# linhthi/BLISS-GNN

Measured on AMD Instinct MI355X. Metric: steps/sec (train step: sample_blocks + gather + SAGE fwd/bwd + Adam + exp3), reddit-like, higher is better.
Workload: dtype bf16

## Files before the change

### bliss_gnn_amd/_lib.py

```python
import ctypes as C
import os

_HERE = os.path.dirname(os.path.abspath(__file__))
LIB_PATH = os.path.join(_HERE, "libbliss_gnn.so")

EINVAL = -1
MODE_BANDIT, MODE_LADIES, MODE_UNIFORM_NODES, MODE_PARTIALS = 0, 1, 4, 8
WIDE_MAX_K = 16384
NR_MAX_FANOUT = 1024
WN_RAW, WN_EXP3 = 0, 1

ERR_BITS = {
    1: "frontier larger than 2^31-1 edges",
    2: "candidate capacity exceeded / seed id out of range",
    4: "kept-node capacity exceeded",
    8: "block-edge capacity exceeded",
    16: "non-finite or negative weight reached an exact reduction",
    32: "exact sum left its fixed-point range",
    64: "seed capacity exceeded",
    128: "random stream ran short / generator made no progress",
    256: "a cross-stream flag never came (bliss_flag_wait timed out)",
}


# ... 259 lines not shown
    "bliss_spmm_bwd": [_P, _P, _P, _P, _P, _P, _P, _I64, _I32, _P, _I32, _I32, C.c_int, _P, _I64, C.c_int, _P, _P],
    "bliss_spmm_max_fwd": [_P, _P, _P, _P, _P, _I64, _I32, _P, _I32, _I32, _P, _I64, _P, _I64, _P, _P],
    "bliss_spmm_max_bwd": [_P, _P, _P, _P, _P, _P, _I64, _P, _I64, _I32, _P, _I32, _I32, _P, _I64, _P, _P],
    "bliss_spmm_max_bwd_relu": [_P, _P, _P, _P, _P, _P, _I64, _P, _I64, _P, _I64, _I32, _P, _I32, _I32, _P, _I64, _P, _P],
    "bliss_spmm_self_fwd": [_P, _P, _P, _P, _P, _I64, _P, _I64, _I32, _P, _P, _I32, _I32, _P, _I64, _P, _P],
    "bliss_spmm_self_bwd": [_P, _P, _P, _P, _P, _P, _P, _I64, _I32, _I32, _P, _P, _I32, _I32, _P, _I64, _P, _P],
    "bliss_sddmm_dot": [_P, _P, _P, _P, _I32, _P, _I64, _P, _I64, _P, _I64, _I32, _I32, _P, _I32, _P],
    "bliss_lstm_tile_rows": [],
    "bliss_lstm_agg_fwd": [_P, _P, _P, _P, _I64, _P, _I64, _P, _P, _I32, _P, _P, _I32, _I32, _P, _I64, _P, _P, _P, _P],
    "bliss_lstm_agg_bwd": [_P, _P, _I64, _P, _I64, _P, _P, _I32, _P, _P, _I32, _I32, _P, _P],
    "bliss_lstm_edge_reduce": [_P, _P, _P, _P, _I32, _P, _I32, _I32, _P, _I64, _P],
    "bliss_block_transpose": [_P, _P, _I32, _I32, _I32, _P, _P, _P, _I64, _P],
    "bliss_spmm_chunk_edges": [_I32],
    "bliss_sage_epilogue_fwd": [_P, _I64, _P, _I64, _I32, _I32, _F, C.c_uint32, _P, _P, _I64, _P, _P],
    "bliss_sage_epilogue_bwd": [_P, _I64, _P, _I64, _I32, _I32, _F, _P, _I64, _P],
    "bliss_gat_chunk_edges": [],
    "bliss_graph_prepare": [_P, _P, _I64, _I32, C.c_int, _P, _P, _P, _P, _P, _P, _I64, _P],
    "bliss_exp3_update": [C.POINTER(Graph), _P, _P, _P, _P, _P, _P, _P, _P, _P, _P, _P, _P, _I32, _P, _I32, _F, _P, _P, C.c_int, _P, _P],
    "bliss_exp3_step": [C.POINTER(Graph), _P, C.POINTER(Exp3Block), _I32, _F, _P, _P],
    "bliss_exp3_normalize_global_rows": [C.POINTER(Exp3Block), _I32, _I64, _P, _I64, _P],
    "bliss_exp3_update_blocks": [C.POINTER(Graph), _P, C.POINTER(Exp3Block), _I32, _F, _P, _P],
    "bliss_exp3_apply": [_P, _P, _P, _P, _P, _I32, _P, _P],
    "bliss_exp3_normalize": [_P, _I64, _P, _P, _P, _P],
    "bliss_row_sum": [_P, _I64, _P, _P],
    "bliss_gat_logits": [_P, _P, _P, _I32, _P, _I64, _P, _I32, _I32, _F, _P, _P],
    "bliss_sage_dgrad": [C.POINTER(DGrad), _P],
    "bliss_sage_wgrad": [C.POINTER(WGrad), _I32, _P, _I64, _P],
    "bliss_gat_dgrad": [C.POINTER(DGrad), _P],
    "bliss_dgrad_wide": [C.POINTER(DGrad), _P],
    "bliss_gat_glue_fwd": [C.POINTER(GatGlue), _P],
# ... 105 lines not shown
```

### bliss_gnn_amd/csrc/prof.h

```cpp
#pragma once
#include <hip/hip_runtime.h>

enum BlissKernelId {
  BK_SEG_SCAN = 0, BK_PASS1, BK_PASS2, BK_CHUNK_SCAN, BK_PASS3, BK_CAND_FINALIZE, BK_POISSON_SCALE, BK_SELECT1, BK_SELECT2,
  BK_BLOCK1, BK_INDPTR_SCAN, BK_BLOCK2, BK_CLEANUP, BK_MT19937, BK_SPMM_FWD, BK_SPMM_BWD, BK_EMBED_NORM, BK_EXP3_UPDATE,
  BK_EXP3_APPLY, BK_NORMALIZE, BK_ROW_SUM, BK_NORM_EDATA, BK_TRANSPOSE, BK_SPMM_FIXUP, BK_SPMM_MAX_FWD, BK_SPMM_MAX_FIXUP,
  BK_SPMM_MAX_BWD, BK_SPMM_MAX_BWD_FIXUP, BK_COL_SUMS, BK_BIN_SCATTER, BK_BIN_REDUCE, BK_BITMAP_SCAN, BK_CAND_NUMBER,
  BK_SPMM_SELF_FWD, BK_SPMM_SELF_FIXUP, BK_SPMM_SELF_BWD, BK_SPMM_SELF_BWD_FIXUP,
  BK_LSTM_AGG_FWD, BK_LSTM_AGG_BWD, BK_LSTM_EDGE_REDUCE,
  BK_SDDMM_DOT,
  BK_SPMM_MAX_BWD_RELU, BK_SPMM_MAX_BWD_RELU_FIXUP, BK_COUNT
};

extern int g_bliss_prof_sel;
void bliss_prof_begin(int id, hipStream_t st);
void bliss_prof_end(int id, hipStream_t st);

#define PROF_LAUNCH(id, st, ...)                                              \
  do {                                                                        \
    const bool p_ = (g_bliss_prof_sel == -1 || g_bliss_prof_sel == (id));    \
    if (p_) bliss_prof_begin((id), (st));                                     \
    __VA_ARGS__;                                                              \
    if (p_) bliss_prof_end((id), (st));                                       \
  } while (0)
// ... 1 lines not shown
```

### bliss_gnn_amd/csrc/prof.hip

```cpp
#include "prof.h"
#include "bliss_gnn.h"
#include <mutex>
#include <vector>

int g_bliss_prof_sel = -2;

namespace {
struct Pair { hipEvent_t a, b; int id; };
std::mutex g_mu;
std::vector<Pair> g_open, g_free;
double g_ms[BK_COUNT];
long long g_n[BK_COUNT];
const char* kNames[BK_COUNT] = {
  "k_seg_scan", "k_frontier_pass1", "k_frontier_pass2", "k_chunk_scan", "k_frontier_pass3", "k_cand_finalize", "k_poisson_scale",
  "k_select_pass1", "k_select_pass2", "k_block_pass1", "k_indptr_scan", "k_block_pass2", "k_cleanup", "k_mt19937_uniform",
  "k_spmm_fwd", "k_spmm_bwd", "k_embed_norm", "k_exp3_update", "k_exp3_apply", "k_normalize_row", "k_row_sum",
  "k_normalized_edata", "k_block_transpose", "k_spmm_fixup", "k_spmm_max", "k_spmm_max_fixup", "k_spmm_max_bwd",
  "k_spmm_max_bwd_fixup", "k_col_sums", "k_bin_scatter", "k_bin_reduce", "k_bitmap_scan", "k_cand_number",
  "k_spmm_self", "k_spmm_self_fixup", "k_spmm_self_bwd", "k_spmm_self_bwd_fixup",
  "k_lstm_agg_fwd", "k_lstm_agg_bwd", "k_lstm_edge_reduce", "k_sddmm_dot",
  "k_spmm_max_bwd_relu", "k_spmm_max_bwd_relu_fixup"};
thread_local Pair t_cur;

void drain_locked() {
  for (auto& p : g_open) {
    (void)hipEventSynchronize(p.b);
    float ms = 0.f;
    if (hipEventElapsedTime(&ms, p.a, p.b) == hipSuccess) { g_ms[p.id] += ms; g_n[p.id] += 1; }
    g_free.push_back(p);
  }
  g_open.clear();
}
}

void bliss_prof_begin(int id, hipStream_t st) {
// ... 47 lines not shown
```

### bliss_gnn_amd/csrc/spmm.hip

```cpp
#include "common.cuh"
#include "spmm_walk.cuh"
#include "bliss_gnn.h"
#include "prof.h"

namespace {

using namespace spmm_walk;

#define SP_TPB 256

template <bool BWD>
struct SagePolicy {
  const int* blk_indptr;
  int mean;
  __device__ __forceinline__ float coef(float c, int s, int d) const {
    if (BWD && mean) c = c / (float)max(blk_indptr[d + 1] - blk_indptr[d], 1);
    return c;
  }
  __device__ __forceinline__ float scale(int r, int rb, int re) const {
    return (!BWD && mean) ? 1.0f / (float)max(re - rb, 1) : 1.0f;
  }
};

template <bool VEC4, bool OUT_F32, bool BWD>
// ... 61 lines not shown
  __builtin_amdgcn_fence(__ATOMIC_RELEASE, "wavefront");
  __builtin_amdgcn_wave_barrier();
  float s = 0.f;
  if (norm_vec4) {
    for (int c = lane * 4; c < dim; c += 256) {
      const float a = bf2f(sh[c]), b = bf2f(sh[c + 1]), cc = bf2f(sh[c + 2]), d = bf2f(sh[c + 3]);
      s += a * a; s += b * b; s += cc * cc; s += d * d;
    }
  } else {
    for (int c = lane; c < dim; c += 64) { const float a = bf2f(sh[c]); s += a * a; }
  }
  for (int d = 32; d >= 1; d >>= 1) s += __shfl_xor(s, d);
  if (lane == 0) norm_out[row] = f2bf(sqrtf(s));
}

template <bool VEC4, bool NORM4>
__global__ void __launch_bounds__(SP_TPB) k_sage_epilogue(const bf16_t* __restrict__ a, int64_t a_stride, const bf16_t* __restrict__ b,
                                                         int64_t b_stride, int n_rows, int dim, uint32_t drop_thresh, float scale,
                                                         uint32_t seed, unsigned long long* ctr, bf16_t* __restrict__ out,
                                                         int64_t out_stride, bf16_t* __restrict__ norm_out) {
  const int lane = lane_id();
  const int row = blockIdx.x * (SP_TPB / 64) + (threadIdx.x >> 6);
  const uint32_t c = drop_thresh ? (uint32_t)__hip_atomic_load(ctr, __ATOMIC_RELAXED, __HIP_MEMORY_SCOPE_AGENT) : 0u;
  if (row < n_rows) {
    const bf16_t *pa = a + row * a_stride, *pb = b + row * b_stride;
    bf16_t* po = out + row * out_stride;
    float s = 0.f;
    static_assert(NORM4 || !VEC4, "8-byte accesses imply the vec4 order");
    constexpr int W = NORM4 ? 4 : 1;
    for (int col = lane * W; col < dim; col += 64 * W) {
      float v[W];
      if (VEC4) {
        const f4 x = load4(pa + col), y = load4(pb + col);
        v[0] = x.x + y.x; v[1 % W] = x.y + y.y; v[2 % W] = x.z + y.z; v[3 % W] = x.w + y.w;
      } else {
#pragma unroll
        for (int i = 0; i < W; ++i) v[i] = bf2f(pa[col + i]) + bf2f(pb[col + i]);
      }
#pragma unroll
      for (int i = 0; i < W; ++i) {
        float t = rbf(v[i]);
        t = t > 0.f ? t : 0.f;
        if (drop_thresh) {
          const bool keep = drop_hash(seed, c, (uint32_t)(row * dim + col + i)) >= drop_thresh;
          t = keep ? rbf(t * scale) : 0.f;
        }
        v[i] = t;
        s += t * t;
      }
      if (VEC4) {
        uint2 o;
        o.x = (uint32_t)f2bf(v[0]) | ((uint32_t)f2bf(v[1 % W]) << 16);
        o.y = (uint32_t)f2bf(v[2 % W]) | ((uint32_t)f2bf(v[3 % W]) << 16);
        *reinterpret_cast<uint2*>(po + col) = o;
      } else {
#pragma unroll
        for (int i = 0; i < W; ++i) po[col + i] = f2bf(v[i]);
      }
    }
    for (int d = 32; d >= 1; d >>= 1) s += __shfl_xor(s, d);
    if (lane == 0 && norm_out) norm_out[row] = f2bf(sqrtf(s));
  }
  if (drop_thresh) {
    __syncthreads();
    if (threadIdx.x == 0) {
      const unsigned G = gridDim.x < 64u ? gridDim.x : 64u, g = blockIdx.x % G;
      const unsigned long long members = (gridDim.x - g + G - 1) / G;
      if (atomicAdd(ctr + 2 + g, 1ull) == members - 1) {
        __hip_atomic_store(ctr + 2 + g, 0ull, __ATOMIC_RELAXED, __HIP_MEMORY_SCOPE_AGENT);
        if (atomicAdd(ctr + 1, 1ull) == (unsigned long long)G - 1) {
          __hip_atomic_store(ctr + 1, 0ull, __ATOMIC_RELAXED, __HIP_MEMORY_SCOPE_AGENT);
          atomicAdd(ctr, 1ull);
        }
      }
    }
  }
}

template <bool VEC4>
__global__ void __launch_bounds__(SP_TPB) k_sage_epilogue_bwd(const bf16_t* __restrict__ dout, int64_t d_stride, const bf16_t* __restrict__ out,
                                                             int64_t out_stride, int n_rows, int dim, float scale,
                                                             bf16_t* __restrict__ din, int64_t din_stride) {
  const int lane = lane_id();
  const int row = blockIdx.x * (SP_TPB / 64) + (threadIdx.x >> 6);
  if (row >= n_rows) return;
  constexpr int W = VEC4 ? 4 : 1;
  for (int col = lane * W; col < dim; col += 64 * W) {
    if (VEC4) {
      const f4 g = load4(dout + row * d_stride + col), o = load4(out + row * out_stride + col);
      f4 r;
      r.x = o.x > 0.f ? g.x * scale : 0.f; r.y = o.y > 0.f ? g.y * scale : 0.f;
      r.z = o.z > 0.f ? g.z * scale : 0.f; r.w = o.w > 0.f ? g.w * scale : 0.f;
      store4<false>(din, row * din_stride + col, r);
    } else {
      const float g = bf2f(dout[row * d_stride + col]);
      din[row * din_stride + col] = f2bf(bf2f(out[row * out_stride + col]) > 0.f ? g * scale : 0.f);
    }
  }
}

template <bool BWD>
int launch_spmm(const int* row_ptr, const int* t_edge, const int* src, const int* dst, const int* blk_indptr, const void* w,
                const void* h, int64_t h_stride, int n_rows, const int* nnz_dev, int nnz, int dim, int mean, void* out,
                int64_t out_stride, int out_fp32, float* part, hipStream_t st) {
  if (n_rows <= 0 || dim <= 0) return 0;
  const int EC = spmm_chunk_edges(nnz);
  if (nnz > EC && !part) return BLISS_EINVAL;
  const bool vec4 = (dim % 4 == 0) && (h_stride % 4 == 0) && (out_stride % 4 == 0) &&
                    (((uintptr_t)h) % 8 == 0) && (((uintptr_t)out) % (out_fp32 ? 16 : 8) == 0);
  const int nchunks = nnz > 0 ? (nnz + EC - 1) / EC : 1;
  dim3 grid((nchunks + SP_TPB / 64 - 1) / (SP_TPB / 64)), block(SP_TPB), gfix((n_rows + SP_TPB / 64 - 1) / (SP_TPB / 64));
#define GO(V, F) PROF_LAUNCH(BWD ? BK_SPMM_BWD : BK_SPMM_FWD, st, k_spmm<V, F, BWD><<<grid, block, 0, st>>>(row_ptr, t_edge, src, dst, blk_indptr, (const bf16_t*)w, (const bf16_t*)h, h_stride, n_rows, nnz_dev, nnz, dim, mean, out, out_stride, part, EC))
  if (vec4) { if (out_fp32) GO(true, true); else GO(true, false); }
  else      { if (out_fp32) GO(false, true); else GO(false, false); }
#undef GO
  {
    const bool fv = vec4 && (((uintptr_t)part) % 16 == 0);
#define FIX(F, V) PROF_LAUNCH(BK_SPMM_FIXUP, st, k_spmm_fixup<F, BWD, V><<<gfix, block, 0, st>>>(row_ptr, n_rows, dim, mean, part, out, out_stride, EC))
    if (out_fp32) { if (fv) FIX(true, true); else FIX(true, false); }
    else          { if (fv) FIX(false, true); else FIX(false, false); }
#undef FIX
  }
  return (int)hipGetLastError();
}

}

extern "C" {

int bliss_spmm_chunk_edges(int32_t nnz_bound) { return spmm_chunk_edges(nnz_bound); }

// ... 15 lines not shown
}

int bliss_sage_epilogue_fwd(const void* a, int64_t a_stride, const void* b, int64_t b_stride, int32_t n_rows, int32_t dim,
                            float p_drop, uint32_t seed, uint64_t* ctr, void* out, int64_t out_stride, void* norm_out, void* stream) {
  if (!a || !b || !out || n_rows < 0 || dim <= 0 || !(p_drop >= 0.f && p_drop < 1.f) || (p_drop > 0.f && !ctr)) return BLISS_EINVAL;
  if (n_rows == 0) return 0;
  const bool v4 = dim % 4 == 0 && a_stride % 4 == 0 && b_stride % 4 == 0 && out_stride % 4 == 0 && ((uintptr_t)a) % 8 == 0 &&
                  ((uintptr_t)b) % 8 == 0 && ((uintptr_t)out) % 8 == 0;
  const uint32_t thresh = p_drop > 0.f ? (uint32_t)((double)p_drop * 4294967296.0) : 0u;
  const float scale = p_drop > 0.f ? 1.0f / (1.0f - p_drop) : 1.0f;
  hipStream_t st = (hipStream_t)stream;
  const int grid = (n_rows + SP_TPB / 64 - 1) / (SP_TPB / 64);
  const bool n4 = dim % 4 == 0 && out_stride % 4 == 0 && ((uintptr_t)out) % 8 == 0;
#define GO(V, N) k_sage_epilogue<V, N><<<grid, SP_TPB, 0, st>>>((const bf16_t*)a, a_stride, (const bf16_t*)b, b_stride, n_rows, dim, thresh, scale, \
                                                              seed, (unsigned long long*)ctr, (bf16_t*)out, out_stride, (bf16_t*)norm_out)
  if (v4) GO(true, true); else if (n4) GO(false, true); else GO(false, false);
#undef GO
  return (int)hipGetLastError();
}

int bliss_sage_epilogue_bwd(const void* dout, int64_t dout_stride, const void* out, int64_t out_stride, int32_t n_rows, int32_t dim,
                            float p_drop, void* din, int64_t din_stride, void* stream) {
  if (!dout || !out || !din || n_rows < 0 || dim <= 0 || !(p_drop >= 0.f && p_drop < 1.f)) return BLISS_EINVAL;
  if (n_rows == 0) return 0;
  const bool v4 = dim % 4 == 0 && dout_stride % 4 == 0 && out_stride % 4 == 0 && din_stride % 4 == 0 && ((uintptr_t)dout) % 8 == 0 &&
                  ((uintptr_t)out) % 8 == 0 && ((uintptr_t)din) % 8 == 0;
  const float scale = p_drop > 0.f ? 1.0f / (1.0f - p_drop) : 1.0f;
  hipStream_t st = (hipStream_t)stream;
  const int grid = (n_rows + SP_TPB / 64 - 1) / (SP_TPB / 64);
  if (v4) k_sage_epilogue_bwd<true><<<grid, SP_TPB, 0, st>>>((const bf16_t*)dout, dout_stride, (const bf16_t*)out, out_stride, n_rows, dim, scale,
// ... 36 lines not shown
```

### bliss_gnn_amd/csrc/spmm_walk.cuh

```cuda
#pragma once
#include "common.cuh"

namespace spmm_walk {

struct f4 { float x, y, z, w; };

__device__ __forceinline__ int bcast_i(int v, int j) { return __builtin_amdgcn_readlane(v, j); }
__device__ __forceinline__ float bcast_f(float v, int j) { return __int_as_float(__builtin_amdgcn_readlane(__float_as_int(v), j)); }

__device__ __forceinline__ f4 load4(const bf16_t* p) {
  uint2 v = *reinterpret_cast<const uint2*>(p);
  f4 r;
  r.x = __uint_as_float(v.x << 16); r.y = __uint_as_float(v.x & 0xffff0000u);
  r.z = __uint_as_float(v.y << 16); r.w = __uint_as_float(v.y & 0xffff0000u);
  return r;
}

template <bool OUT_F32>
__device__ __forceinline__ void store4(void* out, int64_t off, f4 a) {
  if (OUT_F32) {
    *reinterpret_cast<float4*>((float*)out + off) = make_float4(a.x, a.y, a.z, a.w);
  } else {
    uint2 v;
    v.x = (uint32_t)f2bf(a.x) | ((uint32_t)f2bf(a.y) << 16);
    v.y = (uint32_t)f2bf(a.z) | ((uint32_t)f2bf(a.w) << 16);
    *reinterpret_cast<uint2*>((bf16_t*)out + off) = v;
  }
}

template <bool VEC4, bool OUT_F32>
__device__ __forceinline__ void store_row(void* out, int64_t off, f4 a, float scale) {
  a.x *= scale; a.y *= scale; a.z *= scale; a.w *= scale;
  if (VEC4) store4<OUT_F32>(out, off, a);
  else if (OUT_F32) ((float*)out)[off] = a.x;
  else ((bf16_t*)out)[off] = f2bf(a.x);
}

__host__ __device__ inline int spmm_chunk_edges(int nnz) { return nnz >= 200000 ? 64 : (nnz >= 50000 ? 32 : 16); }

template <bool VEC4, bool OUT_F32, bool BWD, class Policy>
__device__ __forceinline__ void chunk(const Policy pol, int ci, int nnz, int EC, const int* __restrict__ row_ptr,
                                      const int* __restrict__ t_edge, const int* __restrict__ src, const int* __restrict__ dst,
                                      const bf16_t* __restrict__ w, const bf16_t* __restrict__ h, int64_t h_stride, int dim,
                                      void* out, int64_t out_stride, float* __restrict__ part) {
  const int lane = lane_id();
  const int c0 = ci * EC, c1 = min(nnz, c0 + EC), cnt = c1 - c0;
  int my_row = -1, my_n = 0;
  float my_c = 0.f;
  if (lane < cnt) {
    const int e = BWD ? t_edge[c0 + lane] : c0 + lane;
    const int s = src[e], d = dst[e];
    my_row = BWD ? s : d;
    my_n = BWD ? d : s;
    my_c = pol.coef(w ? bf2f(w[e]) : 1.0f, s, d);
  }
  constexpr int W = VEC4 ? 4 : 1;
  const f4 zero = {0.f, 0.f, 0.f, 0.f};
  for (int col0 = 0; col0 < dim; col0 += 64 * W) {
    const int col = col0 + lane * W;
    const bool act = col < dim;
    auto flush = [&](int r, f4 acc) {
      const int rb = row_ptr[r], re = row_ptr[r + 1];
      const bool starts = rb >= c0, ends = re <= c1;
      if (!act) return;
      if (starts && ends) {
        store_row<VEC4, OUT_F32>(out, r * out_stride + col, acc, pol.scale(r, rb, re));
      } else {
        float* q = part + ((int64_t)ci * 2 + (starts ? 1 : 0)) * dim + col;
        q[0] = acc.x;
        if (VEC4) { q[1] = acc.y; q[2] = acc.z; q[3] = acc.w; }
      }
    };
    if (cnt == 0) continue;
    int cur = bcast_i(my_row, 0);
    f4 acc = zero;
    for (int j = 0; j < cnt;) {
      const int r = bcast_i(my_row, j);
      if (r != cur) { flush(cur, acc); acc = zero; cur = r; }
      const int run = __popcll(__ballot(my_row == r && lane >= j));
      const int end = j + run;
      for (; j + 4 <= end; j += 4) {
        int n0 = bcast_i(my_n, j), n1 = bcast_i(my_n, j + 1), n2 = bcast_i(my_n, j + 2), n3 = bcast_i(my_n, j + 3);
        float k0 = bcast_f(my_c, j), k1 = bcast_f(my_c, j + 1), k2 = bcast_f(my_c, j + 2), k3 = bcast_f(my_c, j + 3);
        if (act) {
          if (VEC4) {
            f4 a0 = load4(h + n0 * h_stride + col), a1 = load4(h + n1 * h_stride + col);
            f4 a2 = load4(h + n2 * h_stride + col), a3 = load4(h + n3 * h_stride + col);
            acc.x += k0 * a0.x; acc.y += k0 * a0.y; acc.z += k0 * a0.z; acc.w += k0 * a0.w;
            acc.x += k1 * a1.x; acc.y += k1 * a1.y; acc.z += k1 * a1.z; acc.w += k1 * a1.w;
            acc.x += k2 * a2.x; acc.y += k2 * a2.y; acc.z += k2 * a2.z; acc.w += k2 * a2.w;
            acc.x += k3 * a3.x; acc.y += k3 * a3.y; acc.z += k3 * a3.z; acc.w += k3 * a3.w;
          } else {
            float a0 = bf2f(h[n0 * h_stride + col]), a1 = bf2f(h[n1 * h_stride + col]);
            float a2 = bf2f(h[n2 * h_stride + col]), a3 = bf2f(h[n3 * h_stride + col]);
            acc.x += k0 * a0; acc.x += k1 * a1; acc.x += k2 * a2; acc.x += k3 * a3;
          }
        }
      }
      for (; j < end; ++j) {
        int n0 = bcast_i(my_n, j);
        float k0 = bcast_f(my_c, j);
        if (act) {
          if (VEC4) {
            f4 a0 = load4(h + n0 * h_stride + col);
            acc.x += k0 * a0.x; acc.y += k0 * a0.y; acc.z += k0 * a0.z; acc.w += k0 * a0.w;
          } else acc.x += k0 * bf2f(h[n0 * h_stride + col]);
        }
      }
    }
    flush(cur, acc);
  }
}

template <bool VEC4, bool OUT_F32, class Policy>
__device__ __forceinline__ void fixup(const Policy pol, int r, const int* __restrict__ row_ptr, int dim, const float* __restrict__ part,
                                      void* out, int64_t out_stride, int EC) {
  const int lane = lane_id();
  const int rb = row_ptr[r], re = row_ptr[r + 1];
  constexpr int W = VEC4 ? 4 : 1;
  const f4 zero = {0.f, 0.f, 0.f, 0.f};
  if (re <= rb) {
// ... 26 lines not shown
```

### bliss_gnn_amd/model.py

```python
import torch
import torch.nn as nn

from .nn import TILE_KINDS, SAGEConv, SAGEGCNConv, SAGELSTMConv, embed_norm, sage_epilogue


def _gathered_norm(blocks, x):
    fn = getattr(blocks[0].srcdata, "row_norm_of", None) if len(blocks) else None
    return fn(x) if fn is not None else None


class SAGE(nn.Module):

    SAGE_TRANSFORMS = ("auto", "wide", "tile")
    SAGE_AGGREGATORS = ("mean", "pool", "gcn")

    def __init__(self, in_feats, n_hidden, n_classes, n_layers, activation, dropout, transforms="auto", aggregator_type="mean"):
        super().__init__()
        if transforms not in self.SAGE_TRANSFORMS:
            raise ValueError("transforms must be one of %r, not %r" % (self.SAGE_TRANSFORMS, transforms))
        if aggregator_type not in self.SAGE_AGGREGATORS:
            raise NotImplementedError("SAGE: aggregator_type must be one of %r, not %r%s" % (
                self.SAGE_AGGREGATORS, aggregator_type,
                " (the 'lstm' aggregator is the model SAGELSTM: DESIGN.md section 37)" if aggregator_type == "lstm" else ""))
        if aggregator_type != "mean" and transforms == "wide":
# ... 139 lines not shown
        return self._gcn_dstate[key]

    def _layers_gcn_tile(self, blocks, h, norm, lo, hi):
        from .nn import sage_gcn_tile
        n_layers = len(self.layers)
        for l in range(lo, hi):
            layer, block = self.layers[l], blocks[l]
            last = l == n_layers - 1
            block.srcdata["embed_norm"] = embed_norm(h) if norm is None else norm
            ew = block.edata["edge_weights"] if "edge_weights" in block.edata else None
            p = float(self.dropout.p) if (self.training and not last) else 0.0
            h, norm = sage_gcn_tile(block, h, ew, layer, not last, p, self._gcn_drop_state(l, h.device) if p > 0 else None, not last)
        return h, norm

    def _layers_mfma(self, blocks, h, norm, lo, hi, parts=False):
        from .nn import LazyRows, _SageLinearPair, sage_agg_dual, weighted_aggregate
        n_layers = len(self.layers)
        for l in range(lo, hi):
            layer, block = self.layers[l], blocks[l]
            last = l == n_layers - 1
            S_b, K_b = block.num_dst_nodes(), block.num_src_nodes()
            cd = block._counts_dev.data_ptr() if block._nnz_ptr else 0
            src_dev, dst_dev = (cd + 12, cd) if cd else (0, 0)
            ew = block.edata["edge_weights"] if "edge_weights" in block.edata else None
            p = self.dropout.p if (self.training and not last) else 0.0
            ctr, seed = self._dropout_state(l, h.device) if p > 0 else (None, 0)
            fc_n, fc_s = layer.fc_neigh, layer.fc_self
            if layer._in_src_feats > layer._out_feats:
                table, ids = (h.table, h.ids) if isinstance(h, LazyRows) else (h, None)
                z, y, _rows, in_norm = _SageLinearPair.apply(table, ids, fc_n.weight, fc_s.weight, fc_s.bias, K_b, S_b, src_dev, dst_dev,
                                                             self.transforms == "wide")
                block.srcdata["embed_norm"] = in_norm if norm is None else norm
                agg = weighted_aggregate(block, z, ew, mean=True)
                if last:
                    h, norm = ((y, agg) if parts else y + agg), None
                else:
                    h, norm = sage_epilogue(y, agg, p, ctr, seed)
            else:
                if isinstance(h, LazyRows):
                    h = h.materialize()
                block.srcdata["embed_norm"] = embed_norm(h) if norm is None else norm
                h, norm = sage_agg_dual(block, h, ew, fc_n.weight, fc_s.weight, fc_s.bias, not last, p, ctr, seed, dst_dev)
                if last:
                    norm = None
        return h, norm

    def _layers_plain(self, blocks, h, norm, lo, hi):
        for l in range(lo, hi):
            layer, block = self.layers[l], blocks[l]
            block.srcdata["embed_norm"] = embed_norm(h) if norm is None else norm
            norm = None
            ew = block.edata["edge_weights"] if "edge_weights" in block.edata else None
# ... 533 lines not shown
```

### bliss_gnn_amd/nn.py

```python
import torch
import torch.nn as nn

from . import _lib
from ._engine import _stream, spmm_partials


def embed_norm(h):
    from . import ops
    h = h.detach()
    if h.dtype != torch.bfloat16:
        h = h.bfloat16()
    if h.stride(1) != 1:
        h = h.contiguous()
    return ops.embed_norm(h)


def _wait_block(block):
    r = getattr(block, "_ready", None)
    if r is not None:
        _lib.check(_lib.lib.bliss_flag_wait(r[0], r[1], _stream()), "bliss_flag_wait")
        block._ready = None


def _aggregate_operands(block, h, edge_weight):
# ... 103 lines not shown
        (out,) = ctx.saved_tensors
        if dout is None:
            return None, None, None, None, None
        dout = dout.contiguous()
        if dout.dtype != torch.bfloat16:
            dout = dout.bfloat16()
        din = torch.empty_like(out)
        _lib.check(_lib.lib.bliss_sage_epilogue_bwd(dout.data_ptr(), dout.stride(0), out.data_ptr(), out.stride(0), out.shape[0],
                                                    out.shape[1], ctx.p, din.data_ptr(), din.stride(0), _stream()),
                   "bliss_sage_epilogue_bwd")
        return din, din, None, None, None


def sage_epilogue(self_out, neigh, p, ctr, seed):
    return _SageEpilogue.apply(self_out, neigh, p, ctr, seed)


_row_ids = {}


def _identity_ids(n, device):
    key = (int(n), str(device))
    if key not in _row_ids:
        _row_ids[key] = torch.arange(int(n), dtype=torch.int32, device=device)
    return _row_ids[key]


def _live_word(n_rows_dev, device):
    if not (torch.is_tensor(n_rows_dev) and n_rows_dev.dtype == torch.int32 and n_rows_dev.numel() == 1 and n_rows_dev.device == device):
        raise ValueError("n_rows_dev: one int32 word on the logits' device")
# ... 1836 lines not shown
```

### include/bliss_gnn.h

```cpp
#ifndef BLISS_GNN_H
#define BLISS_GNN_H
#include <stdint.h>

#ifdef __cplusplus
extern "C" {
#endif

#define BLISS_EINVAL (-1)

#define BLISS_MODE_BANDIT 0
#define BLISS_MODE_LADIES 1
#define BLISS_ROWSUM_SLOTS 32
#define BLISS_NORM_SCRATCH (2 + 3 * BLISS_ROWSUM_SLOTS)
#define BLISS_MODE_UNIFORM_NODES 4
#define BLISS_MODE_PARTIALS 8

typedef struct {
  const int64_t* indptr;
  const int32_t* indices;
  const int32_t* eid;
  int32_t num_nodes;
  int64_t num_edges;
} bliss_graph_t;

// ... 315 lines not shown
int bliss_lstm_agg_fwd(const int32_t* indptr, const int32_t* src, const void* w, const void* p, int64_t p_stride, const void* w_hh,
                       int64_t w_hh_stride, const void* b_ih, const void* b_hh, int32_t n_dst, const int32_t* n_dst_dev,
                       const int32_t* nnz_dev, int32_t nnz, int32_t dim, void* out, int64_t out_stride, float* gates, float* cell,
                       void* hprev, void* stream);
int bliss_lstm_agg_bwd(const int32_t* indptr, const void* gout, int64_t gout_stride, const void* w_hh_t, int64_t w_hh_t_stride,
                       const float* gates, const float* cell, int32_t n_dst, const int32_t* n_dst_dev, const int32_t* nnz_dev,
                       int32_t nnz, int32_t dim, void* dgate, void* stream);
int bliss_lstm_edge_reduce(const int32_t* t_indptr, const int32_t* t_edge, const void* w, const void* dgate, int32_t n_src,
                           const int32_t* nnz_dev, int32_t nnz, int32_t dim, void* dp, int64_t dp_stride, void* stream);

int bliss_sage_epilogue_fwd(const void* a, int64_t a_stride, const void* b, int64_t b_stride, int32_t n_rows, int32_t dim,
                            float p_drop, uint32_t seed, uint64_t* ctr, void* out, int64_t out_stride, void* norm_out, void* stream);
int bliss_sage_epilogue_bwd(const void* dout, int64_t dout_stride, const void* out, int64_t out_stride, int32_t n_rows, int32_t dim,
                            float p_drop, void* din, int64_t din_stride, void* stream);

int64_t bliss_block_transpose_temp_bytes(int32_t cap_b, int32_t n_src_cap);
int bliss_block_transpose(const int32_t* src, const int32_t* nnz_dev, int32_t nnz, int32_t cap_b, int32_t n_src_cap,
                          int32_t* t_indptr, int32_t* t_edge, void* temp, int64_t temp_bytes, void* stream);

int64_t bliss_graph_prepare_capacity(int64_t n_edges, int32_t num_nodes, int undirected);
int64_t bliss_graph_prepare_temp_bytes(int64_t n_edges, int32_t num_nodes, int undirected);
int bliss_graph_prepare(const int32_t* coo_src, const int32_t* coo_dst, int64_t n_edges, int32_t num_nodes, int undirected,
                        int64_t* indptr, int32_t* indices, int32_t* eid, int64_t* n_out, int32_t* err, void* temp,
                        int64_t temp_bytes, void* stream);

int bliss_exp3_update(const bliss_graph_t* g, const void* edge_w_pos, void* w_pos, int64_t* row_sum,
                      const int32_t* blk_indptr, const int32_t* blk_src, const int32_t* blk_dst,
                      const int32_t* blk_pos, const void* q_ij, const void* node_prob, const void* embed_norm,
                      const void* alpha_or_null, const int32_t* dst_nid, int32_t n_dst, const int32_t* n_edges_dev,
                      int32_t edges_bound, float delta_f, void* rewards_out, void* factor_out, int apply,
// ... 160 lines not shown
```

Baseline: 1589.

## Fuse SpMM fixup into SAGE epilogue and batch gather loads in SpMM walk

Adds a rowfinish kernel that folds the SpMM chunk-partials fixup into the SAGE epilogue (add, ReLU, dropout, norm), so non-final SAGE layers skip the separate fixup launch and one extra pass over the aggregate. The SpMM chunk walk now issues NB=16 neighbour-row loads up front, pinned with empty asm barriers, before accumulating, to expose more memory-level parallelism. It also drops the run-length ballot logic. Costs are more registers per thread for the batched loads, and some wasted loads on short chunks because out-of-range slots clamp to the last edge.

```diff
diff --git a/bliss_gnn_amd/_lib.py b/bliss_gnn_amd/_lib.py
--- a/bliss_gnn_amd/_lib.py
+++ b/bliss_gnn_amd/_lib.py
@@ -297,6 +297,8 @@
     "bliss_spmm_chunk_edges": [_I32],
     "bliss_sage_epilogue_fwd": [_P, _I64, _P, _I64, _I32, _I32, _F, C.c_uint32, _P, _P, _I64, _P, _P],
     "bliss_sage_epilogue_bwd": [_P, _I64, _P, _I64, _I32, _I32, _F, _P, _I64, _P],
+    "bliss_spmm_rowfinish_fwd": [_P, _P, _P, _P, _P, _I64, _I32, _P, _I32, _I32, C.c_int, _P, _I64, _P, _P, _I64, _F, C.c_uint32, _P, _P,
+                                 _I64, _P, _P],
     "bliss_gat_chunk_edges": [],
     "bliss_graph_prepare": [_P, _P, _I64, _I32, C.c_int, _P, _P, _P, _P, _P, _P, _I64, _P],
     "bliss_exp3_update": [C.POINTER(Graph), _P, _P, _P, _P, _P, _P, _P, _P, _P, _P, _P, _P, _I32, _P, _I32, _F, _P, _P, C.c_int, _P, _P],
diff --git a/bliss_gnn_amd/csrc/prof.h b/bliss_gnn_amd/csrc/prof.h
--- a/bliss_gnn_amd/csrc/prof.h
+++ b/bliss_gnn_amd/csrc/prof.h
@@ -7,7 +7,7 @@
   BK_EXP3_APPLY, BK_NORMALIZE, BK_ROW_SUM, BK_NORM_EDATA, BK_TRANSPOSE, BK_SPMM_FIXUP, BK_SPMM_MAX_FWD, BK_SPMM_MAX_FIXUP,
   BK_SPMM_MAX_BWD, BK_SPMM_MAX_BWD_FIXUP, BK_COL_SUMS, BK_BIN_SCATTER, BK_BIN_REDUCE, BK_BITMAP_SCAN, BK_CAND_NUMBER,
   BK_SPMM_SELF_FWD, BK_SPMM_SELF_FIXUP, BK_SPMM_SELF_BWD, BK_SPMM_SELF_BWD_FIXUP,
-  BK_LSTM_AGG_FWD, BK_LSTM_AGG_BWD, BK_LSTM_EDGE_REDUCE,
+  BK_LSTM_AGG_FWD, BK_LSTM_AGG_BWD, BK_LSTM_EDGE_REDUCE, BK_SPMM_ROWFINISH,
   BK_SDDMM_DOT,
   BK_SPMM_MAX_BWD_RELU, BK_SPMM_MAX_BWD_RELU_FIXUP, BK_COUNT
 };
diff --git a/bliss_gnn_amd/csrc/prof.hip b/bliss_gnn_amd/csrc/prof.hip
--- a/bliss_gnn_amd/csrc/prof.hip
+++ b/bliss_gnn_amd/csrc/prof.hip
@@ -18,7 +18,7 @@
   "k_normalized_edata", "k_block_transpose", "k_spmm_fixup", "k_spmm_max", "k_spmm_max_fixup", "k_spmm_max_bwd",
   "k_spmm_max_bwd_fixup", "k_col_sums", "k_bin_scatter", "k_bin_reduce", "k_bitmap_scan", "k_cand_number",
   "k_spmm_self", "k_spmm_self_fixup", "k_spmm_self_bwd", "k_spmm_self_bwd_fixup",
-  "k_lstm_agg_fwd", "k_lstm_agg_bwd", "k_lstm_edge_reduce", "k_sddmm_dot",
+  "k_lstm_agg_fwd", "k_lstm_agg_bwd", "k_lstm_edge_reduce", "k_spmm_rowfinish", "k_sddmm_dot",
   "k_spmm_max_bwd_relu", "k_spmm_max_bwd_relu_fixup"};
 thread_local Pair t_cur;
 
diff --git a/bliss_gnn_amd/csrc/spmm.hip b/bliss_gnn_amd/csrc/spmm.hip
--- a/bliss_gnn_amd/csrc/spmm.hip
+++ b/bliss_gnn_amd/csrc/spmm.hip
@@ -99,67 +99,140 @@
   if (lane == 0) norm_out[row] = f2bf(sqrtf(s));
 }
 
+template <bool VEC4, bool NORM4, class Nb>
+__device__ __forceinline__ void sage_epilogue_row(const bf16_t* __restrict__ pa, const Nb nb, int row, int dim, uint32_t drop_thresh,
+                                                  float scale, uint32_t seed, uint32_t c, bf16_t* __restrict__ po,
+                                                  bf16_t* __restrict__ norm_out) {
+  const int lane = lane_id();
+  float s = 0.f;
+  static_assert(NORM4 || !VEC4, "8-byte accesses imply the vec4 order");
+  constexpr int W = NORM4 ? 4 : 1;
+  for (int col = lane * W; col < dim; col += 64 * W) {
+    float v[W], y[W];
+    nb(col, y);
+    if (VEC4) {
+      const f4 x = load4(pa + col);
+      v[0] = x.x + y[0]; v[1 % W] = x.y + y[1 % W]; v[2 % W] = x.z + y[2 % W]; v[3 % W] = x.w + y[3 % W];
+    } else {
+#pragma unroll
+      for (int i = 0; i < W; ++i) v[i] = bf2f(pa[col + i]) + y[i];
+    }
+#pragma unroll
+    for (int i = 0; i < W; ++i) {
+      float t = rbf(v[i]);
+      t = t > 0.f ? t : 0.f;
+      if (drop_thresh) {
+        const bool keep = drop_hash(seed, c, (uint32_t)(row * dim + col + i)) >= drop_thresh;
+        t = keep ? rbf(t * scale) : 0.f;
+      }
+      v[i] = t;
+      s += t * t;
+    }
+    if (VEC4) {
+      uint2 o;
+      o.x = (uint32_t)f2bf(v[0]) | ((uint32_t)f2bf(v[1 % W]) << 16);
+      o.y = (uint32_t)f2bf(v[2 % W]) | ((uint32_t)f2bf(v[3 % W]) << 16);
+      *reinterpret_cast<uint2*>(po + col) = o;
+    } else {
+#pragma unroll
+      for (int i = 0; i < W; ++i) po[col + i] = f2bf(v[i]);
+    }
+  }
+  for (int d = 32; d >= 1; d >>= 1) s += __shfl_xor(s, d);
+  if (lane == 0 && norm_out) norm_out[row] = f2bf(sqrtf(s));
+}
+
+__device__ __forceinline__ void sage_epilogue_ticket(unsigned long long* ctr) {
+  __syncthreads();
+  if (threadIdx.x == 0) {
+    const unsigned G = gridDim.x < 64u ? gridDim.x : 64u, g = blockIdx.x % G;
+    const unsigned long long members = (gridDim.x - g + G - 1) / G;
+    if (atomicAdd(ctr + 2 + g, 1ull) == members - 1) {
+      __hip_atomic_store(ctr + 2 + g, 0ull, __ATOMIC_RELAXED, __HIP_MEMORY_SCOPE_AGENT);
+      if (atomicAdd(ctr + 1, 1ull) == (unsigned long long)G - 1) {
+        __hip_atomic_store(ctr + 1, 0ull, __ATOMIC_RELAXED, __HIP_MEMORY_SCOPE_AGENT);
+        atomicAdd(ctr, 1ull);
+      }
+    }
+  }
+}
+
 template <bool VEC4, bool NORM4>
 __global__ void __launch_bounds__(SP_TPB) k_sage_epilogue(const bf16_t* __restrict__ a, int64_t a_stride, const bf16_t* __restrict__ b,
                                                          int64_t b_stride, int n_rows, int dim, uint32_t drop_thresh, float scale,
                                                          uint32_t seed, unsigned long long* ctr, bf16_t* __restrict__ out,
                                                          int64_t out_stride, bf16_t* __restrict__ norm_out) {
-  const int lane = lane_id();
   const int row = blockIdx.x * (SP_TPB / 64) + (threadIdx.x >> 6);
   const uint32_t c = drop_thresh ? (uint32_t)__hip_atomic_load(ctr, __ATOMIC_RELAXED, __HIP_MEMORY_SCOPE_AGENT) : 0u;
   if (row < n_rows) {
-    const bf16_t *pa = a + row * a_stride, *pb = b + row * b_stride;
-    bf16_t* po = out + row * out_stride;
-    float s = 0.f;
-    static_assert(NORM4 || !VEC4, "8-byte accesses imply the vec4 order");
     constexpr int W = NORM4 ? 4 : 1;
-    for (int col = lane * W; col < dim; col += 64 * W) {
-      float v[W];
+    const bf16_t* pb = b + row * b_stride;
+    auto nb = [&](int col, float (&y)[W]) {
       if (VEC4) {
-        const f4 x = load4(pa + col), y = load4(pb + col);
-        v[0] = x.x + y.x; v[1 % W] = x.y + y.y; v[2 % W] = x.z + y.z; v[3 % W] = x.w + y.w;
+        const f4 t = load4(pb + col);
+        y[0] = t.x; y[1 % W] = t.y; y[2 % W] = t.z; y[3 % W] = t.w;
       } else {
 #pragma unroll
-        for (int i = 0; i < W; ++i) v[i] = bf2f(pa[col + i]) + bf2f(pb[col + i]);
+        for (int i = 0; i < W; ++i) y[i] = bf2f(pb[col + i]);
       }
-#pragma unroll
-      for (int i = 0; i < W; ++i) {
-        float t = rbf(v[i]);
-        t = t > 0.f ? t : 0.f;
-        if (drop_thresh) {
-          const bool keep = drop_hash(seed, c, (uint32_t)(row * dim + col + i)) >= drop_thresh;
-          t = keep ? rbf(t * scale) : 0.f;
+    };
+    sage_epilogue_row<VEC4, NORM4>(a + row * a_stride, nb, row, dim, drop_thresh, scale, seed, c, out + row * out_stride, norm_out);
+  }
+  if (drop_thresh) sage_epilogue_ticket(ctr);
+}
+
+template <bool VEC4, bool NORM4>
+__global__ void __launch_bounds__(SP_TPB) k_spmm_rowfinish(const int* __restrict__ row_ptr, int n_rows, int dim, int mean,
+                                                          const float* __restrict__ part, const bf16_t* __restrict__ agg,
+                                                          int64_t agg_stride, int EC, const bf16_t* __restrict__ a, int64_t a_stride,
+                                                          uint32_t drop_thresh, float scale, uint32_t seed, unsigned long long* ctr,
+                                                          bf16_t* __restrict__ out, int64_t out_stride, bf16_t* __restrict__ norm_out) {
+  const int row = __builtin_amdgcn_readfirstlane(blockIdx.x * (SP_TPB / 64) + (threadIdx.x >> 6));
+  const uint32_t c = drop_thresh ? (uint32_t)__hip_atomic_load(ctr, __ATOMIC_RELAXED, __HIP_MEMORY_SCOPE_AGENT) : 0u;
+  if (row < n_rows) {
+    constexpr int W = NORM4 ? 4 : 1;
+    const int rb = row_ptr[row], re = row_ptr[row + 1];
+    const bool empty = re <= rb;
+    const int c0 = rb / EC, c_end = empty ? c0 : (re - 1) / EC;
+    const float rscale = SagePolicy<false>{nullptr, mean}.scale(row, rb, re);
+    const bf16_t* pg = agg + row * agg_stride;
+    auto nb = [&](int col, float (&y)[W]) {
+      if (empty) {
+#pragma unroll
+        for (int i = 0; i < W; ++i) y[i] = 0.f;
+      } else if (c_end == c0) {
+        if (VEC4) {
+          const f4 t = load4(pg + col);
+          y[0] = t.x; y[1 % W] = t.y; y[2 % W] = t.z; y[3 % W] = t.w;
+        } else {
+#pragma unroll
+          for (int i = 0; i < W; ++i) y[i] = bf2f(pg[col + i]);
         }
-        v[i] = t;
-        s += t * t;
+      } else {
+        float sum[W];
+        if (VEC4) {
+          const float4 t = *reinterpret_cast<const float4*>(part + ((int64_t)c0 * 2 + 1) * dim + col);
+          sum[0] = t.x; sum[1 % W] = t.y; sum[2 % W] = t.z; sum[3 % W] = t.w;
+#pragma unroll 4
+          for (int cc = c0 + 1; cc <= c_end; ++cc) {
+            const float4 u = *reinterpret_cast<const float4*>(part + ((int64_t)cc * 2) * dim + col);
+            sum[0] += u.x; sum[1 % W] += u.y; sum[2 % W] += u.z; sum[3 % W] += u.w;
+          }
+        } else {
+#pragma unroll
+          for (int i = 0; i < W; ++i) sum[i] = part[((int64_t)c0 * 2 + 1) * dim + col + i];
+          for (int cc = c0 + 1; cc <= c_end; ++cc) {
+#pragma unroll
+            for (int i = 0; i < W; ++i) sum[i] += part[((int64_t)cc * 2) * dim + col + i];
+          }
+        }
+#pragma unroll
+        for (int i = 0; i < W; ++i) y[i] = rbf(sum[i] * rscale);
       }
-      if (VEC4) {
-        uint2 o;
-        o.x = (uint32_t)f2bf(v[0]) | ((uint32_t)f2bf(v[1 % W]) << 16);
-        o.y = (uint32_t)f2bf(v[2 % W]) | ((uint32_t)f2bf(v[3 % W]) << 16);
-        *reinterpret_cast<uint2*>(po + col) = o;
-      } else {
-#pragma unroll
-        for (int i = 0; i < W; ++i) po[col + i] = f2bf(v[i]);
-      }
-    }
-    for (int d = 32; d >= 1; d >>= 1) s += __shfl_xor(s, d);
-    if (lane == 0 && norm_out) norm_out[row] = f2bf(sqrtf(s));
-  }
-  if (drop_thresh) {
-    __syncthreads();
-    if (threadIdx.x == 0) {
-      const unsigned G = gridDim.x < 64u ? gridDim.x : 64u, g = blockIdx.x % G;
-      const unsigned long long members = (gridDim.x - g + G - 1) / G;
-      if (atomicAdd(ctr + 2 + g, 1ull) == members - 1) {
-        __hip_atomic_store(ctr + 2 + g, 0ull, __ATOMIC_RELAXED, __HIP_MEMORY_SCOPE_AGENT);
-        if (atomicAdd(ctr + 1, 1ull) == (unsigned long long)G - 1) {
-          __hip_atomic_store(ctr + 1, 0ull, __ATOMIC_RELAXED, __HIP_MEMORY_SCOPE_AGENT);
-          atomicAdd(ctr, 1ull);
-        }
-      }
-    }
-  }
+    };
+    sage_epilogue_row<VEC4, NORM4>(a + row * a_stride, nb, row, dim, drop_thresh, scale, seed, c, out + row * out_stride, norm_out);
+  }
+  if (drop_thresh) sage_epilogue_ticket(ctr);
 }
 
 template <bool VEC4>
@@ -187,7 +260,7 @@
 template <bool BWD>
 int launch_spmm(const int* row_ptr, const int* t_edge, const int* src, const int* dst, const int* blk_indptr, const void* w,
                 const void* h, int64_t h_stride, int n_rows, const int* nnz_dev, int nnz, int dim, int mean, void* out,
-                int64_t out_stride, int out_fp32, float* part, hipStream_t st) {
+                int64_t out_stride, int out_fp32, float* part, hipStream_t st, bool with_fixup = true) {
   if (n_rows <= 0 || dim <= 0) return 0;
   const int EC = spmm_chunk_edges(nnz);
   if (nnz > EC && !part) return BLISS_EINVAL;
@@ -199,7 +272,7 @@
   if (vec4) { if (out_fp32) GO(true, true); else GO(true, false); }
   else      { if (out_fp32) GO(false, true); else GO(false, false); }
 #undef GO
-  {
+  if (with_fixup) {
     const bool fv = vec4 && (((uintptr_t)part) % 16 == 0);
 #define FIX(F, V) PROF_LAUNCH(BK_SPMM_FIXUP, st, k_spmm_fixup<F, BWD, V><<<gfix, block, 0, st>>>(row_ptr, n_rows, dim, mean, part, out, out_stride, EC))
     if (out_fp32) { if (fv) FIX(true, true); else FIX(true, false); }
@@ -245,6 +318,30 @@
   const bool n4 = dim % 4 == 0 && out_stride % 4 == 0 && ((uintptr_t)out) % 8 == 0;
 #define GO(V, N) k_sage_epilogue<V, N><<<grid, SP_TPB, 0, st>>>((const bf16_t*)a, a_stride, (const bf16_t*)b, b_stride, n_rows, dim, thresh, scale, \
                                                               seed, (unsigned long long*)ctr, (bf16_t*)out, out_stride, (bf16_t*)norm_out)
+  if (v4) GO(true, true); else if (n4) GO(false, true); else GO(false, false);
+#undef GO
+  return (int)hipGetLastError();
+}
+
+int bliss_spmm_rowfinish_fwd(const int32_t* indptr, const int32_t* src, const int32_t* dst, const void* w, const void* h,
+                             int64_t h_stride, int32_t n_dst, const int32_t* nnz_dev, int32_t nnz, int32_t dim, int mean, void* agg,
+                             int64_t agg_stride, float* partials, const void* self, int64_t self_stride, float p_drop, uint32_t seed,
+                             uint64_t* ctr, void* out, int64_t out_stride, void* norm_out, void* stream) {
+  if (!indptr || !h || !agg || nnz < 0 || (nnz > 0 && (!src || !dst))) return BLISS_EINVAL;
+  if (!self || !out || n_dst < 0 || dim <= 0 || !(p_drop >= 0.f && p_drop < 1.f) || (p_drop > 0.f && !ctr)) return BLISS_EINVAL;
+  if (n_dst == 0) return 0;
+  hipStream_t st = (hipStream_t)stream;
+  const int rc = launch_spmm<false>(indptr, nullptr, src, dst, nullptr, w, h, h_stride, n_dst, nnz_dev, nnz, dim, mean, agg, agg_stride, 0,
+                                    partials, st, false);
+  if (rc) return rc;
+  const int EC = spmm_chunk_edges(nnz);
+  const bool n4 = dim % 4 == 0 && out_stride % 4 == 0 && ((uintptr_t)out) % 8 == 0;
+  const bool v4 = n4 && self_stride % 4 == 0 && agg_stride % 4 == 0 && ((uintptr_t)self) % 8 == 0 && ((uintptr_t)agg) % 8 == 0 &&
+                  ((uintptr_t)partials) % 16 == 0;
+  const uint32_t thresh = p_drop > 0.f ? (uint32_t)((double)p_drop * 4294967296.0) : 0u;
+  const float scale = p_drop > 0.f ? 1.0f / (1.0f - p_drop) : 1.0f;
+  const int grid = (n_dst + SP_TPB / 64 - 1) / (SP_TPB / 64);
+#define GO(V, N) PROF_LAUNCH(BK_SPMM_ROWFINISH, st, k_spmm_rowfinish<V, N><<<grid, SP_TPB, 0, st>>>(indptr, n_dst, dim, mean, partials, (const bf16_t*)agg, agg_stride, EC, (const bf16_t*)self, self_stride, thresh, scale, seed, (unsigned long long*)ctr, (bf16_t*)out, out_stride, (bf16_t*)norm_out))
   if (v4) GO(true, true); else if (n4) GO(false, true); else GO(false, false);
 #undef GO
   return (int)hipGetLastError();
diff --git a/bliss_gnn_amd/csrc/spmm_walk.cuh b/bliss_gnn_amd/csrc/spmm_walk.cuh
--- a/bliss_gnn_amd/csrc/spmm_walk.cuh
+++ b/bliss_gnn_amd/csrc/spmm_walk.cuh
@@ -38,12 +38,18 @@
 
 __host__ __device__ inline int spmm_chunk_edges(int nnz) { return nnz >= 200000 ? 64 : (nnz >= 50000 ? 32 : 16); }
 
+#ifndef SPMM_WALK_NB
+#define SPMM_WALK_NB 16
+#endif
+constexpr int NB = SPMM_WALK_NB;
+
 template <bool VEC4, bool OUT_F32, bool BWD, class Policy>
-__device__ __forceinline__ void chunk(const Policy pol, int ci, int nnz, int EC, const int* __restrict__ row_ptr,
+__device__ __forceinline__ void chunk(const Policy pol, int ci_wave, int nnz, int EC, const int* __restrict__ row_ptr,
                                       const int* __restrict__ t_edge, const int* __restrict__ src, const int* __restrict__ dst,
                                       const bf16_t* __restrict__ w, const bf16_t* __restrict__ h, int64_t h_stride, int dim,
                                       void* out, int64_t out_stride, float* __restrict__ part) {
   const int lane = lane_id();
+  const int ci = __builtin_amdgcn_readfirstlane(ci_wave);
   const int c0 = ci * EC, c1 = min(nnz, c0 + EC), cnt = c1 - c0;
   int my_row = -1, my_n = 0;
   float my_c = 0.f;
@@ -72,39 +78,41 @@
       }
     };
     if (cnt == 0) continue;
+    const uint32_t coff = (uint32_t)(act ? col : 0) * (uint32_t)sizeof(bf16_t);
     int cur = bcast_i(my_row, 0);
     f4 acc = zero;
-    for (int j = 0; j < cnt;) {
-      const int r = bcast_i(my_row, j);
-      if (r != cur) { flush(cur, acc); acc = zero; cur = r; }
-      const int run = __popcll(__ballot(my_row == r && lane >= j));
-      const int end = j + run;
-      for (; j + 4 <= end; j += 4) {
-        int n0 = bcast_i(my_n, j), n1 = bcast_i(my_n, j + 1), n2 = bcast_i(my_n, j + 2), n3 = bcast_i(my_n, j + 3);
-        float k0 = bcast_f(my_c, j), k1 = bcast_f(my_c, j + 1), k2 = bcast_f(my_c, j + 2), k3 = bcast_f(my_c, j + 3);
-        if (act) {
-          if (VEC4) {
-            f4 a0 = load4(h + n0 * h_stride + col), a1 = load4(h + n1 * h_stride + col);
-            f4 a2 = load4(h + n2 * h_stride + col), a3 = load4(h + n3 * h_stride + col);
-            acc.x += k0 * a0.x; acc.y += k0 * a0.y; acc.z += k0 * a0.z; acc.w += k0 * a0.w;
-            acc.x += k1 * a1.x; acc.y += k1 * a1.y; acc.z += k1 * a1.z; acc.w += k1 * a1.w;
-            acc.x += k2 * a2.x; acc.y += k2 * a2.y; acc.z += k2 * a2.z; acc.w += k2 * a2.w;
-            acc.x += k3 * a3.x; acc.y += k3 * a3.y; acc.z += k3 * a3.z; acc.w += k3 * a3.w;
-          } else {
-            float a0 = bf2f(h[n0 * h_stride + col]), a1 = bf2f(h[n1 * h_stride + col]);
-            float a2 = bf2f(h[n2 * h_stride + col]), a3 = bf2f(h[n3 * h_stride + col]);
-            acc.x += k0 * a0; acc.x += k1 * a1; acc.x += k2 * a2; acc.x += k3 * a3;
-          }
+    for (int j0 = 0; j0 < cnt; j0 += NB) {
+      uint32_t lo[NB], hi[VEC4 ? NB : 1];
+#pragma unroll
+      for (int u = 0; u < NB; ++u) {
+        const int n = bcast_i(my_n, min(j0 + u, cnt - 1));
+        const char* rowp = reinterpret_cast<const char*>(h + n * h_stride);
+        if (VEC4) {
+          const uint2 v = *reinterpret_cast<const uint2*>(rowp + coff);
+          lo[u] = v.x; hi[VEC4 ? u : 0] = v.y;
+        } else {
+          lo[u] = *reinterpret_cast<const bf16_t*>(rowp + coff);
         }
       }
-      for (; j < end; ++j) {
-        int n0 = bcast_i(my_n, j);
-        float k0 = bcast_f(my_c, j);
-        if (act) {
+#pragma unroll
+      for (int u = 0; u < NB; ++u) {
+        asm volatile("" : "+v"(lo[u]));
+        if (VEC4) asm volatile("" : "+v"(hi[VEC4 ? u : 0]));
+      }
+#pragma unroll
+      for (int u = 0; u < NB; ++u) {
+        const int j = j0 + u;
+        if (j < cnt) {
+          const int r = bcast_i(my_row, j);
+          if (r != cur) { flush(cur, acc); acc = zero; cur = r; }
+          const float k = bcast_f(my_c, j);
           if (VEC4) {
-            f4 a0 = load4(h + n0 * h_stride + col);
-            acc.x += k0 * a0.x; acc.y += k0 * a0.y; acc.z += k0 * a0.z; acc.w += k0 * a0.w;
-          } else acc.x += k0 * bf2f(h[n0 * h_stride + col]);
+            const uint32_t x = lo[u], y = hi[VEC4 ? u : 0];
+            acc.x += k * __uint_as_float(x << 16); acc.y += k * __uint_as_float(x & 0xffff0000u);
+            acc.z += k * __uint_as_float(y << 16); acc.w += k * __uint_as_float(y & 0xffff0000u);
+          } else {
+            acc.x += k * __uint_as_float(lo[u] << 16);
+          }
         }
       }
     }
diff --git a/bliss_gnn_amd/model.py b/bliss_gnn_amd/model.py
--- a/bliss_gnn_amd/model.py
+++ b/bliss_gnn_amd/model.py
@@ -177,7 +177,7 @@
         return h, norm
 
     def _layers_mfma(self, blocks, h, norm, lo, hi, parts=False):
-        from .nn import LazyRows, _SageLinearPair, sage_agg_dual, weighted_aggregate
+        from .nn import LazyRows, _SageLinearPair, sage_agg_dual, sage_aggregate_epilogue, weighted_aggregate
         n_layers = len(self.layers)
         for l in range(lo, hi):
             layer, block = self.layers[l], blocks[l]
@@ -194,11 +194,11 @@
                 z, y, _rows, in_norm = _SageLinearPair.apply(table, ids, fc_n.weight, fc_s.weight, fc_s.bias, K_b, S_b, src_dev, dst_dev,
                                                              self.transforms == "wide")
                 block.srcdata["embed_norm"] = in_norm if norm is None else norm
-                agg = weighted_aggregate(block, z, ew, mean=True)
                 if last:
+                    agg = weighted_aggregate(block, z, ew, mean=True)
                     h, norm = ((y, agg) if parts else y + agg), None
                 else:
-                    h, norm = sage_epilogue(y, agg, p, ctr, seed)
+                    h, norm = sage_aggregate_epilogue(block, y, z, ew, p, ctr, seed)
             else:
                 if isinstance(h, LazyRows):
                     h = h.materialize()
diff --git a/bliss_gnn_amd/nn.py b/bliss_gnn_amd/nn.py
--- a/bliss_gnn_amd/nn.py
+++ b/bliss_gnn_amd/nn.py
@@ -1,3 +1,5 @@
+import os
+
 import torch
 import torch.nn as nn
 
@@ -141,6 +143,55 @@
 
 def sage_epilogue(self_out, neigh, p, ctr, seed):
     return _SageEpilogue.apply(self_out, neigh, p, ctr, seed)
+
+
+class _SageAggEpilogue(torch.autograd.Function):
+
+    @staticmethod
+    def forward(ctx, y, z, w, indptr, src, dst, counts, t_indptr, t_edge, p, ctr, seed):
+        ctx.set_materialize_grads(False)
+        y = y.contiguous()
+        n, d = y.shape
+        B = int(src.numel())
+        agg, out = torch.empty_like(y), torch.empty_like(y)
+        norm = torch.empty(n, dtype=torch.bfloat16, device=y.device)
+        part = spmm_partials(B, d, y.device)
+        _lib.check(_lib.lib.bliss_spmm_rowfinish_fwd(
+            indptr.data_ptr(), src.data_ptr(), dst.data_ptr(), 0 if w is None else w.data_ptr(), z.data_ptr(), z.stride(0), n,
+            0 if counts is None else counts.data_ptr() + 16, B, d, 1, agg.data_ptr(), agg.stride(0),
+            0 if part is None else part.data_ptr(), y.data_ptr(), y.stride(0), float(p), int(seed),
+            0 if ctr is None else ctr.data_ptr(), out.data_ptr(), out.stride(0), norm.data_ptr(), _stream()), "bliss_spmm_rowfinish_fwd")
+        ctx.save_for_backward(out, indptr, src, dst, w, counts, t_indptr, t_edge)
+        ctx.p, ctx.n_src = float(p), z.shape[0]
+        ctx.mark_non_differentiable(norm)
+        return out, norm
+
+    @staticmethod
+    def backward(ctx, dout, _dnorm):
+        from . import ops
+        out, indptr, src, dst, w, counts, t_indptr, t_edge = ctx.saved_tensors
+        if dout is None:
+            return (None,) * 12
+        dout = dout.contiguous()
+        if dout.dtype != torch.bfloat16:
+            dout = dout.bfloat16()
+        din = torch.empty_like(out)
+        _lib.check(_lib.lib.bliss_sage_epilogue_bwd(dout.data_ptr(), dout.stride(0), out.data_ptr(), out.stride(0), out.shape[0],
+                                                    out.shape[1], ctx.p, din.data_ptr(), din.stride(0), _stream()),
+                   "bliss_sage_epilogue_bwd")
+        gz = None
+        if ctx.needs_input_grad[1]:
+            gz = ops.spmm_t(t_indptr, t_edge, src, dst, indptr, w, din, ctx.n_src, counts, True)
+        return (din, gz) + (None,) * 10
+
+
+def sage_aggregate_epilogue(block, self_out, z, edge_weight, p, ctr, seed):
+    w_grad = edge_weight is not None and edge_weight.requires_grad and torch.is_grad_enabled()
+    if w_grad or os.environ.get("BLISS_SPMM_ROWFINISH", "1") == "0":
+        return sage_epilogue(self_out, weighted_aggregate(block, z, edge_weight, mean=True), p, ctr, seed)
+    assert self_out.shape == (block.num_dst_nodes(), z.shape[1]) and self_out.dtype == torch.bfloat16
+    z, w, counts, t_indptr, t_edge = _aggregate_operands(block, z, edge_weight)
+    return _SageAggEpilogue.apply(self_out, z, w, block.indptr, block.src, block.dst, counts, t_indptr, t_edge, p, ctr, seed)
 
 
 _row_ids = {}
diff --git a/include/bliss_gnn.h b/include/bliss_gnn.h
--- a/include/bliss_gnn.h
+++ b/include/bliss_gnn.h
@@ -353,6 +353,11 @@
 int bliss_sage_epilogue_bwd(const void* dout, int64_t dout_stride, const void* out, int64_t out_stride, int32_t n_rows, int32_t dim,
                             float p_drop, void* din, int64_t din_stride, void* stream);
 
+int bliss_spmm_rowfinish_fwd(const int32_t* indptr, const int32_t* src, const int32_t* dst, const void* w, const void* h,
+                             int64_t h_stride, int32_t n_dst, const int32_t* nnz_dev, int32_t nnz, int32_t dim, int mean, void* agg,
+                             int64_t agg_stride, float* partials, const void* self, int64_t self_stride, float p_drop, uint32_t seed,
+                             uint64_t* ctr, void* out, int64_t out_stride, void* norm_out, void* stream);
+
 int64_t bliss_block_transpose_temp_bytes(int32_t cap_b, int32_t n_src_cap);
 int bliss_block_transpose(const int32_t* src, const int32_t* nnz_dev, int32_t nnz, int32_t cap_b, int32_t n_src_cap,
                           int32_t* t_indptr, int32_t* t_edge, void* temp, int64_t temp_bytes, void* stream);
```

After: 1605, median of 6. 1.01x the previous value.
